# yangye1098/Speech-Denoising-Diffusion-Model-2

Measured on AMD Instinct MI355X. Metric: denoised audio sec/sec, 1000-step UNetModified2 @16kHz, higher is better.
Workload: dtype bf16; 1 GPU; UNetModified2 config_unet.json, linear 1e-6..1e-3, T=1000, 16x16448-sample chunks per GPU, condition_in; model=UNetModified2, global_batch=16, seq_len=16448, parallelism=dp1, lane_rows=16

## Files before the change

speech-denoising-diffusion-model-2_amd/csrc/conv_common.h:

```cpp
#pragma once
#include <cstdlib>

#include "sddm_common.h"

namespace sddm {

template <typename T> struct Frag;
template <> struct Frag<bf16_t> { bf16x8 v; };
template <> struct Frag<f16_t> { f16x8 v; };
template <> struct Frag<float> { f32x4 lo, hi; };

template <typename T> __device__ __forceinline__ Frag<T> load_frag(const char* p);
template <> __device__ __forceinline__ Frag<bf16_t> load_frag<bf16_t>(const char* p) { return {*(const bf16x8*)p}; }
template <> __device__ __forceinline__ Frag<f16_t> load_frag<f16_t>(const char* p) { return {*(const f16x8*)p}; }
template <> __device__ __forceinline__ Frag<float> load_frag<float>(const char* p) {
  return {*(const f32x4*)p, *(const f32x4*)(p + 16)};
}

__device__ __forceinline__ void mfma_frag(f32x4& acc, const Frag<bf16_t>& a, const Frag<bf16_t>& b) {
  acc = __builtin_amdgcn_mfma_f32_16x16x32_bf16(a.v, b.v, acc, 0, 0, 0);
}
__device__ __forceinline__ void mfma_frag(f32x4& acc, const Frag<f16_t>& a, const Frag<f16_t>& b) {
  acc = __builtin_amdgcn_mfma_f32_16x16x32_f16(a.v, b.v, acc, 0, 0, 0);
}
// ... 23 lines not shown

template <typename T>
__device__ __forceinline__ void transform16(char* dst, const char* src, const float* sc, const float* sh, bool gn) {
  *(f32x4*)dst = transform_vec<T>(*(const f32x4*)src, sc, sh, gn);
}

template <typename T> __device__ __forceinline__ void store4(T* p, float a, float b, float c, float d);
template <> __device__ __forceinline__ void store4<float>(float* p, float a, float b, float c, float d) {
  *(f32x4*)p = f32x4{a, b, c, d};
}
template <> __device__ __forceinline__ void store4<bf16_t>(bf16_t* p, float a, float b, float c, float d) {
  *(bf16x4*)p = bf16x4{(bf16_t)a, (bf16_t)b, (bf16_t)c, (bf16_t)d};
}
template <> __device__ __forceinline__ void store4<f16_t>(f16_t* p, float a, float b, float c, float d) {
  *(f16x4*)p = f16x4{(f16_t)a, (f16_t)b, (f16_t)c, (f16_t)d};
}
typedef float f32x2 __attribute__((ext_vector_type(2)));
template <typename T> __device__ __forceinline__ void store4p(T* p, f32x2 a, f32x2 b) { store4<T>(p, a.x, a.y, b.x, b.y); }
template <> __device__ __forceinline__ void store4p<bf16_t>(bf16_t* p, f32x2 a, f32x2 b) {
  typedef bf16_t bf16x2_t __attribute__((ext_vector_type(2)));
  typedef unsigned int u32x2_t __attribute__((ext_vector_type(2)));
  const bf16x2_t x = __builtin_convertvector(a, bf16x2_t), y = __builtin_convertvector(b, bf16x2_t);
  *(u32x2_t*)p = u32x2_t{__builtin_bit_cast(unsigned int, x), __builtin_bit_cast(unsigned int, y)};
}
template <typename T> __device__ __forceinline__ f32x2 unpack2(T a, T b) { return f32x2{to_f32<T>(a), to_f32<T>(b)}; }
template <typename T> __device__ __forceinline__ f32x4 load4(const T* p);
template <> __device__ __forceinline__ f32x4 load4<float>(const float* p) { return *(const f32x4*)p; }
template <> __device__ __forceinline__ f32x4 load4<bf16_t>(const bf16_t* p) {
  const bf16x4 v = *(const bf16x4*)p;
  return f32x4{(float)v[0], (float)v[1], (float)v[2], (float)v[3]};
}
template <> __device__ __forceinline__ f32x4 load4<f16_t>(const f16_t* p) {
  const f16x4 v = *(const f16x4*)p;
  return f32x4{(float)v[0], (float)v[1], (float)v[2], (float)v[3]};
}
template <typename T> __device__ __forceinline__ float round_t(float v) { return to_f32<T>(from_f32<T>(v)); }

}

namespace sddm {

template <int CTRL> __device__ __forceinline__ float dpp_f32(float x) {
  return __builtin_bit_cast(float, __builtin_amdgcn_update_dpp(0, __builtin_bit_cast(int, x), CTRL, 0xF, 0xF, false));
}
__device__ __forceinline__ float row_sum16(float x) {
  x += dpp_f32<0xB1>(x);
// ... 276 lines not shown
```

speech-denoising-diffusion-model-2_amd/csrc/conv_deep.hip:

```cpp
#include "conv_common.h"
#include "conv_tile_cfg.h"
#include "kernels.h"

namespace sddm {

__device__ __attribute__((aligned(256))) unsigned char g_deep_zero[256];

constexpr int kDeepMaxChunks = 10;

#ifdef SDDM_STAMPS_ISSUE
#define DS_W(a) SDDM_STAMP(a, 1)
#define DS_STG(a) SDDM_STAMP(a, 2)
#define DS_ISSUED(a) SDDM_STAMP(a, 3)
#define DS_LANDED(a) SDDM_STAMP(a, 4)
#define DS_XFORM(a) SDDM_STAMP(a, 5)
#define DS_KLOOP(a) SDDM_STAMP(a, 6)
#define DS_STORED(a) do {} while (0)
#define DS_STATS(a) do {} while (0)
#else
#define DS_W(a) do {} while (0)
#define DS_STG(a) do {} while (0)
#define DS_ISSUED(a) SDDM_STAMP(a, 1)
#define DS_LANDED(a) SDDM_STAMP(a, 2)
#define DS_XFORM(a) SDDM_STAMP(a, 3)
// ... 303 lines not shown
      }
      put(wv);
    }
  } else {
    put(wv);
  }
  lds_sync();

  float sn = 0.f, s1[4], s2[4];
#pragma unroll
  for (int i = 0; i < 4; ++i) { s1[i] = 0.f; s2[i] = 0.f; }
  T* out = (T*)a.out + (size_t)b * img_out * gCout + n0 + ec4;
#pragma unroll
  for (int it = 0; it < EIT; ++it) {
    const int p = it * PPI + tid / TPP;
    if (p < npv) {
      const int py = p / gTW, px = p - py * gTW;
      f32x4 s = *(const f32x4*)(red + p * NBP + ec4);
#pragma unroll
      for (int w = 1; w < SLOTS; ++w) s += *(const f32x4*)(red + (w * MT + p) * NBP + ec4);
      float d[4];
#pragma unroll
      for (int i = 0; i < 4; ++i) d[i] = s[i] + idr[it][i];
      store4<T>(out + ((y0 + py) * gWo + (x0 + px)) * gCout, d[0] + bb[0], d[1] + bb[1], d[2] + bb[2], d[3] + bb[3]);
#pragma unroll
      for (int i = 0; i < 4; ++i) {
        s1[i] += d[i];
        s2[i] += d[i] * d[i];
      }
      sn += 1.f;
    }
  }
  DS_STORED(a);
  if (a.stats) {
    auto wred = [](float x) {
      if constexpr (TPP == 4) x += dpp_f32<0x124>(x);
      if constexpr (TPP <= 8) x += dpp_f32<0x128>(x);
      x += __shfl_xor(x, 16);
      return x + __shfl_xor(x, 32);
    };
    const float tn = wred(sn);
    float t1[4], t2[4];
#pragma unroll
    for (int i = 0; i < 4; ++i) { t1[i] = wred(s1[i]); t2[i] = wred(s2[i]); }
    lds_sync();
    float* xs = red;
    if (lane < TPP)
// ... 135 lines not shown
```

speech-denoising-diffusion-model-2_amd/csrc/conv_strip_impl.h:

```cpp
#pragma once
#include <type_traits>

#ifndef SDDM_ABL_STRIP
#define SDDM_ABL_STRIP 0
#endif
#ifndef SDDM_STRIP_WLD
#define SDDM_STRIP_WLD 1
#endif
#ifndef SDDM_STRIP_WREG
#define SDDM_STRIP_WREG 1
#endif

#include "conv_common.h"
#include "conv_tile_cfg.h"
#include "kernels.h"

namespace sddm {

static constexpr ConvShape kStripShapes[] = {
    {-1, 0, 1, 1, 1, 1, 0, 0, 0, 0, 0, 0, 0, 0, 0, 0, 0},
    {32, 0, 16, 128, 256, 128, 32, 0, 32, 0, 0, 0, 1, 0, 256, 16, 0},
    {32, 0, 16, 128, 256, 128, 32, 0, 32, 0, 0, 1, 1, 0, 256, 16, 0},
    {64, 0, 8, 64, 128, 64, 32, 0, 64, 0, 0, 0, 1, 0, 256, 8, 0},
    {32, 0, 16, 64, 128, 64, 64, 0, 64, 32, 0, 2, 1, 0, 256, 16, 0},
// ... 16 lines not shown
    {32, 0, 64, 128, 512, 128, 32, 32, 32, 0, 0, 0, 1, 0, 256, 64, 1},
    {32, 0, 64, 128, 512, 128, 32, 0, 32, 32, 32, 2, 1, 0, 256, 64, 1},
};
static constexpr int kNStripShapes = (int)(sizeof(kStripShapes) / sizeof(kStripShapes[0]));

__host__ inline bool strip_shape_matches(const ConvShape& c, int nblk, int mpi, int SR, const ConvArgs& a) {
  return c.cfg == nblk && c.nw == mpi && c.nb == SR && c.Ho == a.Ho && c.Wo == a.Wo && c.CA == a.CA && c.CB == a.CB &&
         c.Cout == a.Cout && c.RCA == a.RCA && c.RCB == a.RCB && c.res == a.res_mode &&
         c.gn == (a.gamma != nullptr ? 1 : 0) && c.up == (a.upsample ? 1 : 0) && a.n_tiles == c.Ho / SR &&
         a.Hi == (c.up ? c.Ho / 2 : c.Ho) && a.Wi == (c.up ? c.Wo / 2 : c.Wo);
}

template <typename T, int FC, int W, int CIN, int MPI, int RES, bool GN, int SH>
__global__ __launch_bounds__(MPI * 2) void conv_strip_kernel(ConvArgs a, int SR_) {
  constexpr ConvShape SC = kStripShapes[SH];
  constexpr bool CS = SH > 0;
  SDDM_SHAPE_GEO(SC, CS, false, a)
  const int SR = CS ? SC.nb : SR_;
  (void)gTR; (void)gTW; (void)gTX; (void)gRes; (void)gGN; (void)gWo;
  constexpr int NT = MPI * 2;
  constexpr int NWV = NT / 64;
  constexpr int ES = (int)sizeof(T);
  constexpr int NBLK = 16 * FC, FP = 2;
  constexpr int TR = MPI / W, R = 2 * TR + 2;
  constexpr int UPP = CIN * ES / 16;
  constexpr int UPL = ES / 2;
  constexpr int VE = 16 / ES;
  constexpr int PL = ((W + 2) * 16 + 255) / 256 * 256;
  constexpr int SLOT = UPP * PL;
  constexpr int NCK = CIN / 32;
  constexpr int WPL = NBLK * 16;
  constexpr int WPLANES = NCK * 9 * 4 * UPL;
  constexpr int PB = 64 / UPP;
  constexpr int NU = TR * W * UPP;
  constexpr int UPT = NU / NT;
  constexpr int IU = ((TR + 2) * W * UPP + NT - 1) / NT;
  constexpr int RCKM = 4;
  static_assert(UPP >= 1 && UPP <= 64 && (64 % UPP) == 0, "channel units must divide a wave");
  static_assert(NU % NT == 0, "prefetch must split evenly");
  typedef T vec4 __attribute__((ext_vector_type(4)));
  extern __shared__ __attribute__((aligned(16))) char smem[];

  const int tid = threadIdx.x, lane = tid & 63, wave = tid >> 6, g = lane >> 4;
  int strip, b, zb;
  xcd_block<SDDM_XCD_ZIN != 0>(gNT, gCout / NBLK, strip, b, zb);
  const int n0 = zb * NBLK;
// ... 21 lines not shown
#pragma unroll
  for (int k = 0; k < IU; ++k) {
    const int u = min(tid + k * NT, (TR + 2) * W * UPP - 1);
    const int grp = u >> 6, j = u & 63;
    const int pix = grp * PB + (j % PB), q = j / PB, r = pix / W, x = pix % W;
    const int ry = min(max(y0 - 1 + r, 0), H - 1);
    const int sy = gUp ? ry >> 1 : ry, sx = gUp ? x >> 1 : x;
    const int c0 = q * VE;
    const bool fa = c0 < gCA;
    ini[k] = *(const f32x4*)((fa ? srcAb : srcBb) + ((size_t)sy * gWi + sx) * (fa ? gCA : gCB) + (fa ? c0 : c0 - gCA));
  }
  constexpr int WUN = NBLK * WPLANES, WU = (WUN + NT - 1) / NT;
  constexpr bool WLD = SDDM_STRIP_WLD && WU <= 12;
  constexpr int RUN_MAX = RES == 2 ? NBLK * RCKM * 4 * UPL : 0, RU = (RUN_MAX + NT - 1) / NT;
  const int RUN = NBLK * RPLANES;
  f32x4 wst[WLD ? WU : 1], rst[WLD && RU > 0 ? RU : 1];
  if constexpr (WLD) {
#pragma unroll
    for (int i = 0; i < WU; ++i) {
      const int u0 = tid + i * NT, u = u0 < WUN ? u0 : 0;
      const int co = u % NBLK, pl = u / NBLK;
      const char* src;
      if constexpr (ES == 2) {
        src = (const char*)a.wgt_t + ((size_t)pl * gCout + n0 + co) * 16;
      } else {
        const int ck = pl / (9 * 4 * UPL), rem = pl - ck * 9 * 4 * UPL, tap = rem / (4 * UPL), un = rem - tap * 4 * UPL;
        src = (const char*)a.wgt + ((((size_t)(n0 + co) * NCK + ck) * 9 + tap) * 32) * ES + un * 16;
      }
      wst[i] = *(const f32x4*)src;
    }
    if constexpr (RES == 2) {
#pragma unroll
      for (int i = 0; i < RU; ++i) {
        const int u0 = tid + i * NT, u = u0 < RUN ? u0 : 0;
        const int co = u % NBLK, pl = u / NBLK;
        const char* src = ES == 2 ? (const char*)a.res_wgt_t + ((size_t)pl * gCout + n0 + co) * 16
                                  : (const char*)a.res_wgt + ((size_t)(n0 + co) * RC) * ES + pl * 16;
        rst[i] = *(const f32x4*)src;
      }
    }
  } else {
    for (int u0 = wave * 64; u0 < NBLK * WPLANES; u0 += NT) {
      const int u = u0 + lane;
      const int co = u % NBLK, pl = u / NBLK;
      const char* src;
      if constexpr (ES == 2) {
        src = (const char*)a.wgt_t + ((size_t)pl * gCout + n0 + co) * 16;
      } else {
        const int ck = pl / (9 * 4 * UPL), rem = pl - ck * 9 * 4 * UPL, tap = rem / (4 * UPL), un = rem - tap * 4 * UPL;
        src = (const char*)a.wgt + ((((size_t)(n0 + co) * NCK + ck) * 9 + tap) * 32) * ES + un * 16;
      }
      __builtin_amdgcn_global_load_lds((const __attribute__((address_space(1))) void*)src,
                                       (__attribute__((address_space(3))) void*)(wl + u0 * 16), 16, 0, 0);
    }
    if constexpr (RES == 2) {
      for (int u0 = wave * 64; u0 < NBLK * RPLANES; u0 += NT) {
        const int u = u0 + lane;
        const int co = u % NBLK, pl = u / NBLK;
        const char* src = ES == 2 ? (const char*)a.res_wgt_t + ((size_t)pl * gCout + n0 + co) * 16
                                  : (const char*)a.res_wgt + ((size_t)(n0 + co) * RC) * ES + pl * 16;
        __builtin_amdgcn_global_load_lds((const __attribute__((address_space(1))) void*)src,
                                         (__attribute__((address_space(3))) void*)(rw + u0 * 16), 16, 0, 0);
      }
    }
  }
  for (int u = tid; u < R * UPP * 2; u += NT) {
    const int side = u & 1, pl = u >> 1;
    *(f32x4*)(ring + pl * PL + (side ? (W + 1) : 0) * 16) = f32x4{0.f, 0.f, 0.f, 0.f};
  }
  if (gn) gl.finish(gf, b, gCA, gCB, gsc, gsc + CIN);
  __syncthreads();
  const int t_now = a.t_dev ? *a.t_dev : 0;
  const float* trow = a.temb ? a.temb + (size_t)(a.temb_per_b ? b : t_now) * a.temb_ld : a.bias;
  float badd[FC][4];
#pragma unroll
  for (int fc = 0; fc < FC; ++fc)
#pragma unroll
    for (int i = 0; i < 4; ++i) {
      const int co = n0 + fc * 16 + 4 * g + i;
      const float bv = a.bias[co], tv = trow[co];
      badd[fc][i] = bv + (a.temb ? tv : 0.f);
    }
  float sshift;
  {
    const int cs = n0 + (tid % NBLK);
    const float bv = a.bias[cs], tv = trow[cs];
    sshift = bv + (a.temb ? tv : 0.f);
  }
  const int base = ((y0 - 1) % R + R) % R;
#pragma unroll
  for (int k = 0; k < IU; ++k) {
    const int u = tid + k * NT;
    if (u >= (TR + 2) * W * UPP) break;
    const int grp = u >> 6, j = u & 63;
    const int pix = grp * PB + (j % PB), q = j / PB, r = pix / W, x = pix % W;
    const int ry = y0 - 1 + r;
    f32x4 v = ini[k];
    if (ry < 0 || ry >= H) v = f32x4{0.f, 0.f, 0.f, 0.f};
    else if (gn) v = transform_fast<T>(v, gsc + q * VE, gsc + CIN + q * VE);
    *(f32x4*)(ring + ((base + r) % R) * SLOT + q * PL + (x + 1) * 16) = v;
  }

// ... 37 lines not shown
#pragma unroll
    for (int k = 0; k < UPT; ++k) {
      const int ry = min(y0 + j * TR + 1 + pr[k], H - 1);
      const int sy = gUp ? (ry >> 1) : ry;
      dst[k] = *(const f32x4*)(rsrc_[k] + (unsigned)__umul24((unsigned)sy, rstr[k]));
    }
  };
  auto xform_unit = [&](const f32x4 (&src)[UPT], int j, int k) {
    const int ry = y0 + j * TR + 1 + pr[k];
    f32x4 v = src[k];
    if constexpr (GN) v = transform_lds<T>(v, gsc + cq[k], gsc + CIN + cq[k]);
    return ry >= H ? f32x4{0.f, 0.f, 0.f, 0.f} : v;
  };
  auto store_rows = [&](const f32x4 (&tv)[UPT], int j) {
    const int sb = (base + j * TR + 2) % R;
#pragma unroll
    for (int k = 0; k < UPT; ++k) {
      int sl = sb + pr[k];
      sl = sl >= R ? sl - R : sl;
      *(f32x4*)(ring + (int)__umul24(sl, SLOT) + loff[k]) = tv[k];
    }
  };
  T* outb = (T*)a.out + (size_t)b * H * W * gCout;
  const T* resb = RES == 1 ? (const T*)a.res_src + (size_t)b * H * W * gCout : outb;
  auto issue_res1 = [&](vec4 (&dst)[FP][FC], int it) {
#pragma unroll
    for (int fp = 0; fp < FP; ++fp) {
      const int yy = min(y0 + it * TR, H - TR) + prow[fp];
      const unsigned po = (unsigned)(yy * W * gCout) + __umul24((unsigned)pcol[fp], (unsigned)gCout) + n0 + 4 * g;
#pragma unroll
      for (int fc = 0; fc < FC; ++fc) dst[fp][fc] = *(const vec4*)((const char*)resb + (po * ES + fc * 16 * ES));
    }
  };
  const T* rawAb = RES == 2 ? (const T*)a.rawA + (size_t)b * H * W * gRCA : outb;
  const T* rawBb = (RES == 2 && gRCB) ? (const T*)a.rawB + (size_t)b * H * W * gRCB : rawAb;
  auto issue_res2 = [&](Frag<T> (&dst)[RCKM][FP], int it) {
#pragma unroll
    for (int ck = 0; ck < RCKM; ++ck)
#pragma unroll
      for (int fp = 0; fp < FP; ++fp) {
        const int yy = min(y0 + it * TR, H - TR) + prow[fp];
        const int c0 = min(ck, rck - 1) * 32 + g * 8;
        const int pix = yy * W + pcol[fp];
        const T* sp = c0 < gRCA ? rawAb + ((int)__umul24(pix, gRCA) + c0) : rawBb + ((int)__umul24(pix, gRCB) + (c0 - gRCA));
        dst[ck][fp] = load_frag<T>((const char*)sp);
      }
  };

  f32x2 s1[FC][2], s2[FC][2], bp[FC][2];
#pragma unroll
  for (int fc = 0; fc < FC; ++fc)
#pragma unroll
    for (int h = 0; h < 2; ++h) {
      s1[fc][h] = f32x2{0.f, 0.f};
// ... 53 lines not shown
          for (int fp = 0; fp < FP; ++fp)
            if (!(dbg & 8)) mfma_frag(acc[fp][fc], af, bf[fp]);
        }
#pragma unroll
        for (int k = 0; k < UPT; ++k)
          if (decltype(LX)::value && ck * 9 + tap == k * 9 * NCK / UPT) tv[k] = (dbg & 2) ? fill[k] : xform_unit(fill, it + 1, k);
      }
    }
    if constexpr (RES == 2) {
#pragma unroll
      for (int ck = 0; ck < RCKM; ++ck) {
        if (ck >= rck) break;
#pragma unroll
        for (int fc = 0; fc < FC; ++fc) {
          const Frag<T> af = load_planes<T>(rbase + ck * 4 * UPL * WPL + fc * 256, WPL);
#pragma unroll
          for (int fp = 0; fp < FP; ++fp) mfma_frag(acc[fp][fc], af, r2cur[ck][fp]);
        }
      }
    }
#pragma unroll
    for (int fp = 0; fp < FP; ++fp) {
      const unsigned po = (unsigned)((y + prow[fp]) * W * gCout) + __umul24((unsigned)pcol[fp], (unsigned)gCout);
#pragma unroll
      for (int fc = 0; fc < FC; ++fc) {
        const unsigned co = n0 + fc * 16 + 4 * g;
        f32x2 d0 = f32x2{acc[fp][fc][0], acc[fp][fc][1]}, d1 = f32x2{acc[fp][fc][2], acc[fp][fc][3]};
        if constexpr (RES == 1) {
          d0 += unpack2<T>(r1cur[fp][fc][0], r1cur[fp][fc][1]);
          d1 += unpack2<T>(r1cur[fp][fc][2], r1cur[fp][fc][3]);
        }
        if (!(dbg & 128)) store4p<T>((T*)((char*)outb + (po + co) * ES), d0 + bp[fc][0], d1 + bp[fc][1]);
        s1[fc][0] += d0;
        s1[fc][1] += d1;
        s2[fc][0] = __builtin_elementwise_fma(d0, d0, s2[fc][0]);
        s2[fc][1] = __builtin_elementwise_fma(d1, d1, s2[fc][1]);
      }
    }
    if constexpr (decltype(LX)::value) store_rows(tv, it + 1);
    lds_sync();
  };
  issue_rows(rowsA, 1);
  if constexpr (RES == 1) issue_res1(r1A, 0);
  if constexpr (RES == 2) issue_res2(r2A, 0);
  constexpr int NYOUNG = UPT + (RES == 1 ? FP * FC : 0) + (RES == 2 ? RCKM * FP : 0);
  static_assert(NYOUNG < 64, "vmcnt is a 6-bit counter");
  asm volatile("s_waitcnt vmcnt(%0) lgkmcnt(0)\n\ts_barrier" :: "n"(NYOUNG) : "memory");
  if constexpr (WREG) {
#pragma unroll
    for (int tap = 0; tap < 9; ++tap)
#pragma unroll
      for (int fc = 0; fc < FC; ++fc) wreg[tap][fc] = load_planes<T>(abase + tap * 4 * UPL * WPL + fc * 256, WPL);
  }
  SDDM_STAMP(a, 3);
  using yes = std::integral_constant<bool, true>;
  using no = std::integral_constant<bool, false>;
  for (int it = 0; it < iters - 2; it += 2) {
    body(yes{}, yes{}, it, rowsB, rowsA, r1A, r1B, r2A, r2B);
    body(yes{}, yes{}, it + 1, rowsA, rowsB, r1B, r1A, r2B, r2A);
  }
  body(no{}, yes{}, iters - 2, rowsB, rowsA, r1A, r1B, r2A, r2B);
  body(no{}, no{}, iters - 1, rowsA, rowsB, r1B, r1A, r2B, r2A);

  SDDM_STAMP(a, 4);
  if (a.stats) {
    const float nl = (float)(FP * iters) * 16.f;
#pragma unroll
    for (int fc = 0; fc < FC; ++fc)
#pragma unroll
      for (int i = 0; i < 4; ++i) {
        const float t1 = row_sum16(s1[fc][i >> 1][i & 1]), t2 = row_sum16(s2[fc][i >> 1][i & 1]);
        if ((lane & 15) == 0) {
          float* rr = red + ((wave * NBLK) + fc * 16 + 4 * g + i) * 3;
          rr[0] = nl; rr[1] = t1; rr[2] = t2;
        }
      }
    lds_sync();
    if (tid < NBLK) {
      float n = 0.f, u1 = 0.f, u2 = 0.f;
      for (int w = 0; w < NWV; ++w) {
        const float* rr = red + (w * NBLK + tid) * 3;
        n += rr[0]; u1 += rr[1]; u2 += rr[2];
      }
      float* dst = a.stats + (((size_t)b * gNT + strip) * gCout + n0 + tid) * 2;
      dst[0] = (sshift + u1 / n) * n;
      dst[1] = fmaxf(u2 - u1 * u1 / n, 0.f);
    }
  }
  SDDM_STAMP(a, 6);
  SDDM_STAMP(a, 7);
}

template <typename T, int FC, int W, int CIN, int MPI>
static size_t strip_lds(const ConvArgs& a) {
  constexpr int ES = (int)sizeof(T), NBLK = 16 * FC, TR = MPI / W, R = 2 * TR + 2;
  constexpr int UPP = CIN * ES / 16, PL = ((W + 2) * 16 + 255) / 256 * 256;
// ... 63 lines not shown
```

speech-denoising-diffusion-model-2_amd/csrc/conv_tile.hip:

```cpp
#include "conv_common.h"
#include "conv_tile_cfg.h"
#include "kernels.h"

#ifndef SDDM_TILE_WREG
#define SDDM_TILE_WREG 1
#endif

namespace sddm {

template <typename T, bool S2, int WPX, int WCO, int FP, int FC, int MAXU, int SH>
__global__ __launch_bounds__(64 * WPX * WCO) void conv_tile_kernel(ConvArgs a) {
  constexpr int NWV = WPX * WCO, NT = 64 * NWV;
  constexpr int MT = WPX * FP * 16, NB = WCO * FC * 16;
  constexpr int WCH = 576 * NB;
  static_assert(sizeof(T) == 2, "conv_tile is the 16-bit path");
  typedef T vec4 __attribute__((ext_vector_type(4)));
  extern __shared__ __attribute__((aligned(16))) char smem[];
  constexpr ConvShape SC = kTileShapes[SH];
  constexpr bool CS = SH > 0;
  SDDM_SHAPE_GEO(SC, CS, S2, a)

  const int tid = threadIdx.x, lane = tid & 63, g = lane >> 4, c16 = lane & 15, q = lane & 3;
  const int wv = __builtin_amdgcn_readfirstlane(tid >> 6);
  const int wp = wv % WPX, wc = wv / WPX;
  int tile, b, zb;
  xcd_block<SDDM_XCD_ZIN != 0>(gNT, gCout / NB, tile, b, zb);
  const int n0 = zb * NB;
  const int ty = tile / gTX, tx = tile - ty * gTX;
  const int y0 = ty * gTR, x0 = tx * gTW;
  const int npv = gTR * gTW;
  const int Cin = gCA + gCB, nck = Cin / 32, ckA = gCA / 32;
  const int RC = gRCA + gRCB, rck = gRes == 2 ? RC / 32 : 0, rckA = gRCA / 32;
  const int nk = nck + rck;
  const bool gn = gGN, ident = gRes == 1;
  const TileGeo geo = tile_geo(S2, gTR, gTW, MT, rck > 0);
  const int HC = geo.HC, HE = geo.HE, PLB = geo.PLB;
  const int nbuf = nk > 1 ? 2 : 1;
  char* IB = smem;
  char* WB = IB + nbuf * geo.ibb;
  float* gsc = (float*)(WB + nbuf * WCH);
  const float rHC = 1.0f / (float)HC, rTW = 1.0f / (float)gTW;
  const int img_in = gHi * gWi, img_out = gHo * gWo;
  const T* srcA = (const T*)a.srcA + (size_t)b * img_in * gCA;
  const T* srcB = gCB ? (const T*)a.srcB + (size_t)b * img_in * gCB : srcA;
  const T* rawA = rck ? (const T*)a.rawA + (size_t)b * img_out * gRCA : srcA;
  const T* rawB = (rck && gRCB) ? (const T*)a.rawB + (size_t)b * img_out * gRCB : rawA;
  SDDM_STAMP(a, 0);

  GNLoad gl;
  const GNFuse gf{a.gstA, a.gtilesA, a.gntileA, a.gstB, a.gtilesB, a.gntileB, a.gamma, a.beta, a.groups, a.eps};
  gl.issue(gf, b, gCA, gCB, gn, a.bias);
  const int t_now = a.t_dev ? *a.t_dev : 0;
  const float* trow = a.temb ? a.temb + (size_t)(a.temb_per_b ? b : t_now) * a.temb_ld : a.bias;
  const int cw0 = wc * FC * 16, pw0 = wp * FP * 16;
  float bb[FC][4];
#pragma unroll
  for (int fc = 0; fc < FC; ++fc)
#pragma unroll
    for (int i = 0; i < 4; ++i) {
      const int co = n0 + cw0 + fc * 16 + 4 * g + i;
      const float bv = a.bias[co], tv = trow[co];
      bb[fc][i] = bv + (a.temb ? tv : 0.f);
    }
  float sshift;
  {
    const int cs = n0 + (tid % NB);
    const float bv = a.bias[cs], tv = trow[cs];
    sshift = bv + (a.temb ? tv : 0.f);
  }
  int ppy[FP], ppx[FP];
  bool pok[FP];
#pragma unroll
  for (int fp = 0; fp < FP; ++fp) {
    int p = pw0 + fp * 16 + c16;
    pok[fp] = p < npv;
    if (!pok[fp]) p = 0;
    ppy[fp] = fdivi(p, rTW);
    ppx[fp] = p - ppy[fp] * gTW;
  }
  vec4 r1[FP][FC];
  {
    const T* rs = ident ? (const T*)a.res_src + (size_t)b * img_out * gCout : srcA;
#pragma unroll
    for (int fp = 0; fp < FP; ++fp) {
      const int po = ident ? ((y0 + ppy[fp]) * gWo + (x0 + ppx[fp])) * gCout : 0;
#pragma unroll
      for (int fc = 0; fc < FC; ++fc) r1[fp][fc] = *(const vec4*)(rs + po + (ident ? n0 + cw0 + fc * 16 + 4 * g : 0));
    }
  }
  int spx[MAXU], sof[MAXU];
#pragma unroll
  for (int j = 0; j < MAXU; ++j) {
    const int u = tid + j * NT, s = u >> 2;
    const int hy = fdivi(s, rHC), hx = s - hy * HC;
    int iy, ix, slot;
    bool ok;
    if (S2) {
      iy = 2 * y0 - 1 + hy; ix = 2 * x0 - 1 + hx;
      ok = iy >= 0 && iy < gHi && ix >= 0 && ix < gWi;
      slot = hy * HC + ((hx & 1) ? HE + (hx >> 1) : (hx >> 1));
    } else {
      iy = y0 - 1 + hy; ix = x0 - 1 + hx;
      ok = iy >= 0 && iy < gHo && ix >= 0 && ix < gWo;
      if (gUp) { iy >>= 1; ix >>= 1; }
      slot = s;
    }
    spx[j] = ok ? iy * gWi + ix : -1;
    sof[j] = u < geo.nu3 ? q * PLB + ((slot ^ (q << 1)) << 4) : -1;
  }

// ... 6 lines not shown
#pragma unroll
      for (int j = 0; j < MAXU; ++j) rr[j] = *(const f32x4*)(base + (spx[j] < 0 ? 0 : spx[j] * cs));
    } else {
      const int r = k - nck;
      const bool fa = r < rckA;
      const T* base = (fa ? rawA + r * 32 : rawB + (r - rckA) * 32) + q * 8;
      const int cs = fa ? gRCA : gRCB;
#pragma unroll
      for (int j = 0; j < MAXU; ++j) {
        const int p = (tid + j * NT) >> 2;
        const int py = fdivi(p, rTW), px = p - py * gTW;
        rr[j] = *(const f32x4*)(base + (p < npv ? ((y0 + py) * gWo + (x0 + px)) * cs : 0));
      }
    }
  };
  auto issue_w = [&](int k, int buf) {
    char* dst = WB + buf * WCH;
    const bool res = k >= nck;
    const int nw = (res ? 4 : 36) * NB;
    const char* ws = res ? (const char*)a.res_wgt_t + (size_t)(k - nck) * 4 * gCout * 16
                         : (const char*)a.wgt_t + (size_t)k * 36 * gCout * 16;
    for (int u0 = wv * 64; u0 < nw; u0 += NT) {
      const int u = u0 + lane, r = u / NB, co = u - r * NB;
      glds16(ws + ((size_t)r * gCout + n0 + co) * 16, dst + u0 * 16);
    }
  };
  constexpr bool WR = SDDM_TILE_WREG && (SH > 0 || FP * FC <= 6);
  constexpr int WU = (36 * NB + NT - 1) / NT;
  f32x4 wr[WR ? WU : 1];
  auto load_w = [&](int k) {
    const bool res = k >= nck;
    const int nw = (res ? 4 : 36) * NB;
    const char* ws = res ? (const char*)a.res_wgt_t + (size_t)(k - nck) * 4 * gCout * 16
                         : (const char*)a.wgt_t + (size_t)k * 36 * gCout * 16;
#pragma unroll
    for (int i = 0; i < WU; ++i) {
      const int u = tid + i * NT, uu = u < nw ? u : 0, r = uu / NB, co = uu - r * NB;
      wr[i] = *(const f32x4*)(ws + ((size_t)r * gCout + n0 + co) * 16);
    }
  };
  auto store_w = [&](int k, int buf) {
    const int nw = (k >= nck ? 4 : 36) * NB;
    char* dst = WB + buf * WCH;
#pragma unroll
    for (int i = 0; i < WU; ++i) {
      const int u = tid + i * NT;
      if (u < nw) *(f32x4*)(dst + u * 16) = wr[i];
    }
  };
  auto transform = [&](int k, int buf) {
    char* ib = IB + buf * geo.ibb;
    if (k < nck) {
      float sc[8], sh[8];
      if (gn) {
        const int c = k * 32 + q * 8;
#pragma unroll
        for (int j = 0; j < 8; j += 4) {
          const f32x4 s4 = *(const f32x4*)(gsc + c + j), h4 = *(const f32x4*)(gsc + Cin + c + j);
#pragma unroll
          for (int i = 0; i < 4; ++i) { sc[j + i] = s4[i]; sh[j + i] = h4[i]; }
        }
// ... 86 lines not shown
      if (k + 1 < nk) {
        if (!(dbg & 4)) load_raw(k + 1);
        if (!(dbg & 32)) load_w(k + 1);
      }
      if (!(dbg & 8)) mma(k, cur);
      if (k + 1 < nk) {
        if (!(dbg & 2)) transform(k + 1, nxt);
        if (!(dbg & 32)) store_w(k + 1, nxt);
      }
      lds_sync();
    } else {
      if (k + 1 < nk) {
        if (!(dbg & 4)) load_raw(k + 1);
        if (!(dbg & 32)) issue_w(k + 1, nxt);
      }
      if (!(dbg & 8)) mma(k, cur);
      if (k + 1 < nk && !(dbg & 2)) transform(k + 1, nxt);
      dma_sync();
    }
  }
  SDDM_STAMP(a, 4);

  T* out = (T*)a.out + (size_t)b * img_out * gCout;
  float s1[FC][4], s2[FC][4], nl = 0.f;
#pragma unroll
  for (int fc = 0; fc < FC; ++fc)
#pragma unroll
    for (int i = 0; i < 4; ++i) { s1[fc][i] = 0.f; s2[fc][i] = 0.f; }
#pragma unroll
  for (int fp = 0; fp < FP; ++fp) {
    if (!pok[fp]) continue;
    nl += 1.f;
    const int po = ((y0 + ppy[fp]) * gWo + (x0 + ppx[fp])) * gCout;
#pragma unroll
    for (int fc = 0; fc < FC; ++fc) {
      const int co = n0 + cw0 + fc * 16 + 4 * g;
      float d[4];
#pragma unroll
      for (int i = 0; i < 4; ++i) d[i] = acc[fp][fc][i] + (ident ? to_f32<T>(r1[fp][fc][i]) : 0.f);
      if (!(dbg & 128)) store4<T>(out + po + co, d[0] + bb[fc][0], d[1] + bb[fc][1], d[2] + bb[fc][2], d[3] + bb[fc][3]);
#pragma unroll
      for (int i = 0; i < 4; ++i) {
        s1[fc][i] += d[i];
        s2[fc][i] += d[i] * d[i];
      }
    }
  }
  SDDM_STAMP(a, 5);
  if (a.stats) {
    float* red = (float*)IB;
    const float nr = row_sum16(nl);
#pragma unroll
    for (int fc = 0; fc < FC; ++fc)
#pragma unroll
      for (int i = 0; i < 4; ++i) {
        const float t1 = row_sum16(s1[fc][i]), t2 = row_sum16(s2[fc][i]);
        if (c16 == 0) {
          float* e = red + (wp * NB + cw0 + fc * 16 + 4 * g + i) * 3;
          e[0] = nr; e[1] = t1; e[2] = t2;
        }
      }
    lds_sync();
    if (tid < NB) {
      float n = 0.f, t1 = 0.f, t2 = 0.f;
#pragma unroll
      for (int w = 0; w < WPX; ++w) {
        const float* e = red + (w * NB + tid) * 3;
        n += e[0]; t1 += e[1]; t2 += e[2];
      }
      const int co = tid;
      const float mean = sshift + t1 / n;
      float* dst = a.stats + (((size_t)b * gNT + tile) * gCout + n0 + co) * 2;
      dst[0] = mean * n;
      dst[1] = fmaxf(t2 - t1 * t1 / n, 0.f);
    }
  }
  SDDM_STAMP(a, 6);
  SDDM_STAMP(a, 7);
}

template <int I>
// ... 76 lines not shown
```

speech-denoising-diffusion-model-2_amd/csrc/kernels.hip:

```cpp
#include "sddm_common.h"
#include "kernels.h"
#include "conv_common.h"
#include <algorithm>
#include <type_traits>

namespace sddm {


__global__ __launch_bounds__(256) void embed_kernel(EmbedArgs a) {
  __shared__ float enc[128];
  __shared__ float h1[512];
  __shared__ float h2[128];
  const int r = blockIdx.x, tid = threadIdx.x, D = a.dim, H = a.dim / 2, D4 = 4 * a.dim;
  float nl;
  if (a.noise_levels) nl = a.noise_levels[r];
  else if (a.time_step_mode) nl = (float)r;
  else nl = a.table[r];
  if (tid < D) {
    const float arg = __fmul_rn(nl, a.emb_vec[tid % H]);
    enc[tid] = tid < H ? sinf(arg) : cosf(arg);
  }
  __syncthreads();
  for (int j = tid; j < D4; j += blockDim.x) {
    float s = a.b1[j];
// ... 73 lines not shown
    a.scale[(size_t)b * C + c] = (float)sc;
    a.shift[(size_t)b * C + c] = (float)((double)a.beta[c] - mean * sc);
  }
}

hipError_t launch_gn_finalize(const GNArgs& a, hipStream_t s) {
  hipLaunchKernelGGL(gn_finalize_kernel, dim3(a.G, a.B), dim3(256), 0, s, a);
  return hipGetLastError();
}

template <typename T>
__global__ __launch_bounds__(256) void conv_in_kernel(ConvInArgs a) {
  constexpr int CO = 32;
  constexpr int IMAX = 6 * 130;
  constexpr int NFR = 8;
  __shared__ float img[2][IMAX];
  __shared__ float xs_red[4][CO][2];
  const int b = blockIdx.y, f0 = blockIdx.x * a.TR, tid = threadIdx.x;
  const int lane = tid & 63, wave = tid >> 6, g = lane >> 4;
  if (a.t_dev && blockIdx.x == 0 && blockIdx.y == 0 && tid == 0) *a.t_dev -= 1;
  SDDM_STAMP_AT(a, 0, blockIdx.x + blockIdx.y * (a.F / a.TR));
  const int S = a.S, F = a.F, W = a.W, IW = W + 2, IH = a.TR + 2;
  constexpr int KPL = sizeof(T) == 4 ? 5 : 8;
  float bias[2][4];
#pragma unroll
  for (int fc = 0; fc < 2; ++fc)
#pragma unroll
    for (int i = 0; i < 4; ++i) bias[fc][i] = a.bias[fc * 16 + 4 * g + i];
  float wf[2][KPL];
#pragma unroll
  for (int j = 0; j < KPL; ++j) {
    const int k = sizeof(T) == 4 ? 4 * j + g : 8 * g + j;
    const int kk = k < 18 ? k : 0;
#pragma unroll
    for (int fc = 0; fc < 2; ++fc) wf[fc][j] = a.w[(fc * 16 + (lane & 15)) * 18 + kk];
  }
  {
    const float* c0 = a.cond + (size_t)b * a.N;
    const float* x0 = a.x + (size_t)b * a.N;
    constexpr int IPT = (IMAX + 255) / 256;
    float cv[IPT], xv[IPT];
#pragma unroll
    for (int k = 0; k < IPT; ++k) {
      const int i = min(tid + 256 * k, IH * IW - 1);
      const int r = i / IW, c = i - r * IW, f = f0 - 1 + r, w = c - 1;
      const bool ok = f >= 0 && f < F && w >= 0 && w < W;
      const int n = ok ? f * S + w : 0;
      cv[k] = c0[n];
      xv[k] = x0[n];
      cv[k] = ok ? cv[k] : 0.f;
      xv[k] = ok ? xv[k] : 0.f;
    }
#pragma unroll
    for (int k = 0; k < IPT; ++k) {
      const int i = tid + 256 * k;
      if (i < IH * IW) { img[0][i] = cv[k]; img[1][i] = xv[k]; }
    }
  }
// ... 7 lines not shown
    koff[j] = ch * IMAX + (tap / 3) * IW + (tap % 3);
#pragma unroll
    for (int fc = 0; fc < 2; ++fc) wf[fc][j] = kok[j] ? wf[fc][j] : 0.f;
  }
  f16x8 wh[2], wl[2];
#pragma unroll
  for (int fc = 0; fc < 2; ++fc)
#pragma unroll
    for (int j = 0; j < 8; ++j) {
      const float v = j < KPL ? wf[fc][j] : 0.f;
      wh[fc][j] = (f16_t)v;
      wl[fc][j] = (f16_t)(v - (float)wh[fc][j]);
    }
  f32x2 st1[2][2], st2[2][2], bp[2][2];
#pragma unroll
  for (int fc = 0; fc < 2; ++fc)
#pragma unroll
    for (int h = 0; h < 2; ++h) {
      st1[fc][h] = f32x2{0.f, 0.f};
      st2[fc][h] = f32x2{0.f, 0.f};
      bp[fc][h] = f32x2{bias[fc][2 * h], bias[fc][2 * h + 1]};
    }
  const float rW = 1.0f / (float)W;
  __syncthreads();
  SDDM_STAMP_AT(a, 1, blockIdx.x + blockIdx.y * (a.F / a.TR));
  const float* imgf = &img[0][0];
#pragma unroll 2
  for (int fr = 0; fr < NFR; ++fr) {
    const int p = wave * (NFR * 16) + fr * 16 + (lane & 15);
    const int r = fdivi(p, rW), w = p - r * W;
    const int pb = r * IW + w;
    float xv[KPL];
#pragma unroll
    for (int j = 0; j < KPL; ++j) xv[j] = kok[j] ? imgf[pb + koff[j]] : 0.f;
    f32x4 acc[2];
    if constexpr (sizeof(T) == 4) {
#pragma unroll
      for (int fc = 0; fc < 2; ++fc) {
        acc[fc] = f32x4{0.f, 0.f, 0.f, 0.f};
#pragma unroll
        for (int j = 0; j < KPL; ++j) acc[fc] = __builtin_amdgcn_mfma_f32_16x16x4f32(wf[fc][j], xv[j], acc[fc], 0, 0, 0);
      }
    } else if constexpr (std::is_same<T, bf16_t>::value) {
      f16x8 xh;
#pragma unroll
      for (int j = 0; j < 8; ++j) xh[j] = (f16_t)(j < KPL ? xv[j] : 0.f);
#pragma unroll
      for (int fc = 0; fc < 2; ++fc)
        acc[fc] = __builtin_amdgcn_mfma_f32_16x16x32_f16(wh[fc], xh, f32x4{0.f, 0.f, 0.f, 0.f}, 0, 0, 0);
    } else {
      f16x8 xh, xl;
#pragma unroll
      for (int j = 0; j < 8; ++j) {
        const float v = j < KPL ? xv[j] : 0.f;
        xh[j] = (f16_t)v;
        xl[j] = (f16_t)(v - (float)xh[j]);
      }
#pragma unroll
      for (int fc = 0; fc < 2; ++fc) {
        acc[fc] = __builtin_amdgcn_mfma_f32_16x16x32_f16(wh[fc], xh, f32x4{0.f, 0.f, 0.f, 0.f}, 0, 0, 0);
        acc[fc] = __builtin_amdgcn_mfma_f32_16x16x32_f16(wh[fc], xl, acc[fc], 0, 0, 0);
        acc[fc] = __builtin_amdgcn_mfma_f32_16x16x32_f16(wl[fc], xh, acc[fc], 0, 0, 0);
      }
    }
    T* op = (T*)a.out + (((size_t)b * F + f0 + r) * W + w) * CO;
#pragma unroll
    for (int fc = 0; fc < 2; ++fc) {
      const f32x2 d0 = f32x2{acc[fc][0], acc[fc][1]}, d1 = f32x2{acc[fc][2], acc[fc][3]};
      st1[fc][0] += d0;
      st1[fc][1] += d1;
      st2[fc][0] = __builtin_elementwise_fma(d0, d0, st2[fc][0]);
      st2[fc][1] = __builtin_elementwise_fma(d1, d1, st2[fc][1]);
      store4p<T>(op + fc * 16 + 4 * g, d0 + bp[fc][0], d1 + bp[fc][1]);
    }
  }
  SDDM_STAMP_AT(a, 2, blockIdx.x + blockIdx.y * (a.F / a.TR));
#pragma unroll
  for (int fc = 0; fc < 2; ++fc)
#pragma unroll
    for (int i = 0; i < 4; ++i) {
      const float t1 = row_sum16(st1[fc][i >> 1][i & 1]);
      const float t2 = row_sum16(st2[fc][i >> 1][i & 1]);
      if ((lane & 15) == 0) {
        xs_red[wave][fc * 16 + 4 * g + i][0] = t1;
        xs_red[wave][fc * 16 + 4 * g + i][1] = t2;
      }
    }
  lds_sync();
  SDDM_STAMP_AT(a, 3, blockIdx.x + blockIdx.y * (a.F / a.TR));
  if (tid < CO) {
    const float n = (float)(a.TR * W);
    float S1 = 0.f, S2 = 0.f;
#pragma unroll
    for (int w4 = 0; w4 < 4; ++w4) { S1 += xs_red[w4][tid][0]; S2 += xs_red[w4][tid][1]; }
    float* dst = a.stats + (((size_t)b * (a.F / a.TR) + blockIdx.x) * CO + tid) * 2;
    dst[0] = a.bias[tid] * n + S1;
    dst[1] = fmaxf(S2 - S1 * S1 / n, 0.f);
  }
  SDDM_STAMP_AT(a, 6, blockIdx.x + blockIdx.y * (a.F / a.TR));
  SDDM_STAMP_AT(a, 7, blockIdx.x + blockIdx.y * (a.F / a.TR));
}

hipError_t launch_conv_in(int dtype, const ConvInArgs& a, int B, hipStream_t s) {
  if (a.Cout != 32 || a.TR * a.W != 512 || a.F % a.TR || (a.TR + 2) * (a.W + 2) > 6 * 130) return hipErrorInvalidValue;
  dim3 grid(a.F / a.TR, B);
  if (dtype == DT_F32) hipLaunchKernelGGL(conv_in_kernel<float>, grid, dim3(256), 0, s, a);
  else if (dtype == DT_BF16) hipLaunchKernelGGL(conv_in_kernel<bf16_t>, grid, dim3(256), 0, s, a);
  else hipLaunchKernelGGL(conv_in_kernel<f16_t>, grid, dim3(256), 0, s, a);
// ... 305 lines not shown
```

Measured before the change: 25.07 audio_s/s.

## Permute output channels to pair fragments into 16-byte stores with streaming hints

Remaps which output channels each MFMA fragment computes, so a lane holds 8 adjacent channels across two fragment columns. The conv_in and strip kernels can then emit one 16-byte store where they previously issued two 8-byte stores. Weight, bias, residual and stats indexing are permuted to match. Separately, 16-bit output stores go through buffer or atomic-relaxed stores with a cache-policy bit (write-through or streaming) in the strip and conv_in paths, to cut write-back traffic. The risks are extra register pressure from holding paired values and possible cache side effects when the next layer reads these outputs.

```diff
diff --git a/speech-denoising-diffusion-model-2_amd/csrc/conv_common.h b/speech-denoising-diffusion-model-2_amd/csrc/conv_common.h
--- a/speech-denoising-diffusion-model-2_amd/csrc/conv_common.h
+++ b/speech-denoising-diffusion-model-2_amd/csrc/conv_common.h
@@ -69,6 +69,67 @@
   typedef unsigned int u32x2_t __attribute__((ext_vector_type(2)));
   const bf16x2_t x = __builtin_convertvector(a, bf16x2_t), y = __builtin_convertvector(b, bf16x2_t);
   *(u32x2_t*)p = u32x2_t{__builtin_bit_cast(unsigned int, x), __builtin_bit_cast(unsigned int, y)};
+}
+#ifndef SDDM_WT_STRIP
+#define SDDM_WT_STRIP 1
+#endif
+#ifndef SDDM_WT_TILE
+#define SDDM_WT_TILE 0
+#endif
+#ifndef SDDM_WT_DEEP
+#define SDDM_WT_DEEP 0
+#endif
+#ifndef SDDM_WT_IN
+#define SDDM_WT_IN 1
+#endif
+typedef __attribute__((address_space(1))) unsigned long long gu64_t;
+__device__ __forceinline__ void store8b_wt(void* p, unsigned long long v) {
+  __hip_atomic_store((gu64_t*)p, v, __ATOMIC_RELAXED, __HIP_MEMORY_SCOPE_AGENT);
+}
+template <bool WT, typename T> __device__ __forceinline__ void store4(T* p, float a, float b, float c, float d) {
+  if constexpr (WT && sizeof(T) == 2) {
+    typedef T vec4 __attribute__((ext_vector_type(4)));
+    store8b_wt(p, __builtin_bit_cast(unsigned long long, vec4{(T)a, (T)b, (T)c, (T)d}));
+  } else {
+    store4<T>(p, a, b, c, d);
+  }
+}
+template <bool WT, typename T> __device__ __forceinline__ void store4p(T* p, f32x2 a, f32x2 b) {
+  if constexpr (WT && sizeof(T) == 2) {
+    typedef T vec2 __attribute__((ext_vector_type(2)));
+    typedef unsigned int u32x2_t __attribute__((ext_vector_type(2)));
+    const vec2 x = __builtin_convertvector(a, vec2), y = __builtin_convertvector(b, vec2);
+    store8b_wt(p, __builtin_bit_cast(unsigned long long,
+                                     u32x2_t{__builtin_bit_cast(unsigned int, x), __builtin_bit_cast(unsigned int, y)}));
+  } else {
+    store4p<T>(p, a, b);
+  }
+}
+#ifndef SDDM_ST16_IN
+#define SDDM_ST16_IN 1
+#endif
+#ifndef SDDM_ST16_STRIP
+#define SDDM_ST16_STRIP 1
+#endif
+#ifndef SDDM_ST16_TILE
+#define SDDM_ST16_TILE 0
+#endif
+__host__ __device__ constexpr int pair_channel(int fc, int r) { return 8 * (r / 4) + 4 * (fc & 1) + r % 4 + 32 * (fc / 2); }
+template <bool ST16> __device__ constexpr int slab_channel(int c) { return ST16 ? pair_channel(c >> 4, c & 15) : c; }
+typedef unsigned int u32x4_t __attribute__((ext_vector_type(4)));
+__device__ __forceinline__ __amdgpu_buffer_rsrc_t out_rsrc(void* base, unsigned bytes) {
+  return __builtin_amdgcn_make_buffer_rsrc(base, 0, (int)bytes, 0x00020000);
+}
+template <typename T> __device__ __forceinline__ unsigned int pack2(f32x2 a) {
+  typedef T vec2 __attribute__((ext_vector_type(2)));
+  return __builtin_bit_cast(unsigned int, __builtin_convertvector(a, vec2));
+}
+template <bool WT, typename T>
+__device__ __forceinline__ void store8p(char* base, __amdgpu_buffer_rsrc_t rs, unsigned off, f32x2 a, f32x2 b, f32x2 c, f32x2 d) {
+  static_assert(sizeof(T) == 2, "16-byte stores of 8 channels: 16-bit storage types");
+  const u32x4_t v = u32x4_t{pack2<T>(a), pack2<T>(b), pack2<T>(c), pack2<T>(d)};
+  if constexpr (WT) __builtin_amdgcn_raw_buffer_store_b128(v, rs, (int)off, 0, 16);
+  else *(u32x4_t*)(base + off) = v;
 }
 template <typename T> __device__ __forceinline__ f32x2 unpack2(T a, T b) { return f32x2{to_f32<T>(a), to_f32<T>(b)}; }
 template <typename T> __device__ __forceinline__ f32x4 load4(const T* p);
diff --git a/speech-denoising-diffusion-model-2_amd/csrc/conv_deep.hip b/speech-denoising-diffusion-model-2_amd/csrc/conv_deep.hip
--- a/speech-denoising-diffusion-model-2_amd/csrc/conv_deep.hip
+++ b/speech-denoising-diffusion-model-2_amd/csrc/conv_deep.hip
@@ -349,7 +349,7 @@
       float d[4];
 #pragma unroll
       for (int i = 0; i < 4; ++i) d[i] = s[i] + idr[it][i];
-      store4<T>(out + ((y0 + py) * gWo + (x0 + px)) * gCout, d[0] + bb[0], d[1] + bb[1], d[2] + bb[2], d[3] + bb[3]);
+      store4<SDDM_WT_DEEP != 0, T>(out + ((y0 + py) * gWo + (x0 + px)) * gCout, d[0] + bb[0], d[1] + bb[1], d[2] + bb[2], d[3] + bb[3]);
 #pragma unroll
       for (int i = 0; i < 4; ++i) {
         s1[i] += d[i];
diff --git a/speech-denoising-diffusion-model-2_amd/csrc/conv_strip_impl.h b/speech-denoising-diffusion-model-2_amd/csrc/conv_strip_impl.h
--- a/speech-denoising-diffusion-model-2_amd/csrc/conv_strip_impl.h
+++ b/speech-denoising-diffusion-model-2_amd/csrc/conv_strip_impl.h
@@ -62,6 +62,7 @@
   constexpr int NWV = NT / 64;
   constexpr int ES = (int)sizeof(T);
   constexpr int NBLK = 16 * FC, FP = 2;
+  constexpr bool ST16 = SDDM_ST16_STRIP != 0 && ES == 2 && FC % 2 == 0;
   constexpr int TR = MPI / W, R = 2 * TR + 2;
   constexpr int UPP = CIN * ES / 16;
   constexpr int UPL = ES / 2;
@@ -129,7 +130,7 @@
       const int co = u % NBLK, pl = u / NBLK;
       const char* src;
       if constexpr (ES == 2) {
-        src = (const char*)a.wgt_t + ((size_t)pl * gCout + n0 + co) * 16;
+        src = (const char*)a.wgt_t + ((size_t)pl * gCout + n0 + slab_channel<ST16>(co)) * 16;
       } else {
         const int ck = pl / (9 * 4 * UPL), rem = pl - ck * 9 * 4 * UPL, tap = rem / (4 * UPL), un = rem - tap * 4 * UPL;
         src = (const char*)a.wgt + ((((size_t)(n0 + co) * NCK + ck) * 9 + tap) * 32) * ES + un * 16;
@@ -141,7 +142,7 @@
       for (int i = 0; i < RU; ++i) {
         const int u0 = tid + i * NT, u = u0 < RUN ? u0 : 0;
         const int co = u % NBLK, pl = u / NBLK;
-        const char* src = ES == 2 ? (const char*)a.res_wgt_t + ((size_t)pl * gCout + n0 + co) * 16
+        const char* src = ES == 2 ? (const char*)a.res_wgt_t + ((size_t)pl * gCout + n0 + slab_channel<ST16>(co)) * 16
                                   : (const char*)a.res_wgt + ((size_t)(n0 + co) * RC) * ES + pl * 16;
         rst[i] = *(const f32x4*)src;
       }
@@ -152,7 +153,7 @@
       const int co = u % NBLK, pl = u / NBLK;
       const char* src;
       if constexpr (ES == 2) {
-        src = (const char*)a.wgt_t + ((size_t)pl * gCout + n0 + co) * 16;
+        src = (const char*)a.wgt_t + ((size_t)pl * gCout + n0 + slab_channel<ST16>(co)) * 16;
       } else {
         const int ck = pl / (9 * 4 * UPL), rem = pl - ck * 9 * 4 * UPL, tap = rem / (4 * UPL), un = rem - tap * 4 * UPL;
         src = (const char*)a.wgt + ((((size_t)(n0 + co) * NCK + ck) * 9 + tap) * 32) * ES + un * 16;
@@ -164,7 +165,7 @@
       for (int u0 = wave * 64; u0 < NBLK * RPLANES; u0 += NT) {
         const int u = u0 + lane;
         const int co = u % NBLK, pl = u / NBLK;
-        const char* src = ES == 2 ? (const char*)a.res_wgt_t + ((size_t)pl * gCout + n0 + co) * 16
+        const char* src = ES == 2 ? (const char*)a.res_wgt_t + ((size_t)pl * gCout + n0 + slab_channel<ST16>(co)) * 16
                                   : (const char*)a.res_wgt + ((size_t)(n0 + co) * RC) * ES + pl * 16;
         __builtin_amdgcn_global_load_lds((const __attribute__((address_space(1))) void*)src,
                                          (__attribute__((address_space(3))) void*)(rw + u0 * 16), 16, 0, 0);
@@ -184,7 +185,7 @@
   for (int fc = 0; fc < FC; ++fc)
 #pragma unroll
     for (int i = 0; i < 4; ++i) {
-      const int co = n0 + fc * 16 + 4 * g + i;
+      const int co = n0 + slab_channel<ST16>(fc * 16 + 4 * g + i);
       const float bv = a.bias[co], tv = trow[co];
       badd[fc][i] = bv + (a.temb ? tv : 0.f);
     }
@@ -268,14 +269,17 @@
     }
   };
   T* outb = (T*)a.out + (size_t)b * H * W * gCout;
+  [[maybe_unused]] const __amdgpu_buffer_rsrc_t ors = out_rsrc(outb, (unsigned)(H * W * gCout) * (unsigned)ES);
   const T* resb = RES == 1 ? (const T*)a.res_src + (size_t)b * H * W * gCout : outb;
   auto issue_res1 = [&](vec4 (&dst)[FP][FC], int it) {
 #pragma unroll
     for (int fp = 0; fp < FP; ++fp) {
       const int yy = min(y0 + it * TR, H - TR) + prow[fp];
-      const unsigned po = (unsigned)(yy * W * gCout) + __umul24((unsigned)pcol[fp], (unsigned)gCout) + n0 + 4 * g;
-#pragma unroll
-      for (int fc = 0; fc < FC; ++fc) dst[fp][fc] = *(const vec4*)((const char*)resb + (po * ES + fc * 16 * ES));
+      const unsigned po = (unsigned)(yy * W * gCout) + __umul24((unsigned)pcol[fp], (unsigned)gCout) + n0 +
+                          slab_channel<ST16>(4 * g);
+#pragma unroll
+      for (int fc = 0; fc < FC; ++fc)
+        dst[fp][fc] = *(const vec4*)((const char*)resb + (po * ES + (slab_channel<ST16>(fc * 16) * ES)));
     }
   };
   const T* rawAb = RES == 2 ? (const T*)a.rawA + (size_t)b * H * W * gRCA : outb;
@@ -375,6 +379,7 @@
 #pragma unroll
     for (int fp = 0; fp < FP; ++fp) {
       const unsigned po = (unsigned)((y + prow[fp]) * W * gCout) + __umul24((unsigned)pcol[fp], (unsigned)gCout);
+      [[maybe_unused]] f32x2 pv0, pv1;
 #pragma unroll
       for (int fc = 0; fc < FC; ++fc) {
         const unsigned co = n0 + fc * 16 + 4 * g;
@@ -383,7 +388,18 @@
           d0 += unpack2<T>(r1cur[fp][fc][0], r1cur[fp][fc][1]);
           d1 += unpack2<T>(r1cur[fp][fc][2], r1cur[fp][fc][3]);
         }
-        if (!(dbg & 128)) store4p<T>((T*)((char*)outb + (po + co) * ES), d0 + bp[fc][0], d1 + bp[fc][1]);
+        if constexpr (ST16) {
+          if (fc & 1) {
+            if (!(dbg & 128))
+              store8p<SDDM_WT_STRIP != 0, T>((char*)outb, ors, (po + n0 + (fc / 2) * 32 + 8 * g) * ES, pv0, pv1,
+                                             d0 + bp[fc][0], d1 + bp[fc][1]);
+          } else {
+            pv0 = d0 + bp[fc][0];
+            pv1 = d1 + bp[fc][1];
+          }
+        } else {
+          if (!(dbg & 128)) store4p<SDDM_WT_STRIP != 0, T>((T*)((char*)outb + (po + co) * ES), d0 + bp[fc][0], d1 + bp[fc][1]);
+        }
         s1[fc][0] += d0;
         s1[fc][1] += d1;
         s2[fc][0] = __builtin_elementwise_fma(d0, d0, s2[fc][0]);
@@ -424,7 +440,7 @@
       for (int i = 0; i < 4; ++i) {
         const float t1 = row_sum16(s1[fc][i >> 1][i & 1]), t2 = row_sum16(s2[fc][i >> 1][i & 1]);
         if ((lane & 15) == 0) {
-          float* rr = red + ((wave * NBLK) + fc * 16 + 4 * g + i) * 3;
+          float* rr = red + ((wave * NBLK) + slab_channel<ST16>(fc * 16 + 4 * g + i)) * 3;
           rr[0] = nl; rr[1] = t1; rr[2] = t2;
         }
       }
diff --git a/speech-denoising-diffusion-model-2_amd/csrc/conv_tile.hip b/speech-denoising-diffusion-model-2_amd/csrc/conv_tile.hip
--- a/speech-denoising-diffusion-model-2_amd/csrc/conv_tile.hip
+++ b/speech-denoising-diffusion-model-2_amd/csrc/conv_tile.hip
@@ -14,6 +14,7 @@
   constexpr int MT = WPX * FP * 16, NB = WCO * FC * 16;
   constexpr int WCH = 576 * NB;
   static_assert(sizeof(T) == 2, "conv_tile is the 16-bit path");
+  constexpr bool ST16 = SDDM_ST16_TILE != 0 && FC % 2 == 0;
   typedef T vec4 __attribute__((ext_vector_type(4)));
   extern __shared__ __attribute__((aligned(16))) char smem[];
   constexpr ConvShape SC = kTileShapes[SH];
@@ -58,7 +59,7 @@
   for (int fc = 0; fc < FC; ++fc)
 #pragma unroll
     for (int i = 0; i < 4; ++i) {
-      const int co = n0 + cw0 + fc * 16 + 4 * g + i;
+      const int co = n0 + cw0 + slab_channel<ST16>(fc * 16 + 4 * g + i);
       const float bv = a.bias[co], tv = trow[co];
       bb[fc][i] = bv + (a.temb ? tv : 0.f);
     }
@@ -85,7 +86,7 @@
     for (int fp = 0; fp < FP; ++fp) {
       const int po = ident ? ((y0 + ppy[fp]) * gWo + (x0 + ppx[fp])) * gCout : 0;
 #pragma unroll
-      for (int fc = 0; fc < FC; ++fc) r1[fp][fc] = *(const vec4*)(rs + po + (ident ? n0 + cw0 + fc * 16 + 4 * g : 0));
+      for (int fc = 0; fc < FC; ++fc) r1[fp][fc] = *(const vec4*)(rs + po + (ident ? n0 + cw0 + slab_channel<ST16>(fc * 16 + 4 * g) : 0));
     }
   }
   int spx[MAXU], sof[MAXU];
@@ -138,7 +139,7 @@
                          : (const char*)a.wgt_t + (size_t)k * 36 * gCout * 16;
     for (int u0 = wv * 64; u0 < nw; u0 += NT) {
       const int u = u0 + lane, r = u / NB, co = u - r * NB;
-      glds16(ws + ((size_t)r * gCout + n0 + co) * 16, dst + u0 * 16);
+      glds16(ws + ((size_t)r * gCout + n0 + slab_channel<ST16>(co)) * 16, dst + u0 * 16);
     }
   };
   constexpr bool WR = SDDM_TILE_WREG && (SH > 0 || FP * FC <= 6);
@@ -152,7 +153,7 @@
 #pragma unroll
     for (int i = 0; i < WU; ++i) {
       const int u = tid + i * NT, uu = u < nw ? u : 0, r = uu / NB, co = uu - r * NB;
-      wr[i] = *(const f32x4*)(ws + ((size_t)r * gCout + n0 + co) * 16);
+      wr[i] = *(const f32x4*)(ws + ((size_t)r * gCout + n0 + slab_channel<ST16>(co)) * 16);
     }
   };
   auto store_w = [&](int k, int buf) {
@@ -285,6 +286,7 @@
   SDDM_STAMP(a, 4);
 
   T* out = (T*)a.out + (size_t)b * img_out * gCout;
+  [[maybe_unused]] const __amdgpu_buffer_rsrc_t ors = out_rsrc(out, (unsigned)(img_out * gCout) * (unsigned)sizeof(T));
   float s1[FC][4], s2[FC][4], nl = 0.f;
 #pragma unroll
   for (int fc = 0; fc < FC; ++fc)
@@ -295,13 +297,26 @@
     if (!pok[fp]) continue;
     nl += 1.f;
     const int po = ((y0 + ppy[fp]) * gWo + (x0 + ppx[fp])) * gCout;
+    [[maybe_unused]] f32x2 pv0, pv1;
 #pragma unroll
     for (int fc = 0; fc < FC; ++fc) {
       const int co = n0 + cw0 + fc * 16 + 4 * g;
       float d[4];
 #pragma unroll
       for (int i = 0; i < 4; ++i) d[i] = acc[fp][fc][i] + (ident ? to_f32<T>(r1[fp][fc][i]) : 0.f);
-      if (!(dbg & 128)) store4<T>(out + po + co, d[0] + bb[fc][0], d[1] + bb[fc][1], d[2] + bb[fc][2], d[3] + bb[fc][3]);
+      if constexpr (ST16) {
+        const f32x2 o0 = f32x2{d[0] + bb[fc][0], d[1] + bb[fc][1]}, o1 = f32x2{d[2] + bb[fc][2], d[3] + bb[fc][3]};
+        if (fc & 1) {
+          if (!(dbg & 128))
+            store8p<SDDM_WT_TILE != 0, T>((char*)out, ors, (unsigned)(po + n0 + cw0 + (fc / 2) * 32 + 8 * g) * (unsigned)sizeof(T),
+                                          pv0, pv1, o0, o1);
+        } else {
+          pv0 = o0;
+          pv1 = o1;
+        }
+      } else {
+        if (!(dbg & 128)) store4<SDDM_WT_TILE != 0, T>(out + po + co, d[0] + bb[fc][0], d[1] + bb[fc][1], d[2] + bb[fc][2], d[3] + bb[fc][3]);
+      }
 #pragma unroll
       for (int i = 0; i < 4; ++i) {
         s1[fc][i] += d[i];
@@ -319,7 +334,7 @@
       for (int i = 0; i < 4; ++i) {
         const float t1 = row_sum16(s1[fc][i]), t2 = row_sum16(s2[fc][i]);
         if (c16 == 0) {
-          float* e = red + (wp * NB + cw0 + fc * 16 + 4 * g + i) * 3;
+          float* e = red + (wp * NB + cw0 + slab_channel<ST16>(fc * 16 + 4 * g + i)) * 3;
           e[0] = nr; e[1] = t1; e[2] = t2;
         }
       }
diff --git a/speech-denoising-diffusion-model-2_amd/csrc/kernels.hip b/speech-denoising-diffusion-model-2_amd/csrc/kernels.hip
--- a/speech-denoising-diffusion-model-2_amd/csrc/kernels.hip
+++ b/speech-denoising-diffusion-model-2_amd/csrc/kernels.hip
@@ -119,18 +119,20 @@
   SDDM_STAMP_AT(a, 0, blockIdx.x + blockIdx.y * (a.F / a.TR));
   const int S = a.S, F = a.F, W = a.W, IW = W + 2, IH = a.TR + 2;
   constexpr int KPL = sizeof(T) == 4 ? 5 : 8;
+  constexpr bool ST16 = SDDM_ST16_IN != 0 && sizeof(T) == 2;
+  auto chan = [](int fc, int r) { return ST16 ? pair_channel(fc, r) : fc * 16 + r; };
   float bias[2][4];
 #pragma unroll
   for (int fc = 0; fc < 2; ++fc)
 #pragma unroll
-    for (int i = 0; i < 4; ++i) bias[fc][i] = a.bias[fc * 16 + 4 * g + i];
+    for (int i = 0; i < 4; ++i) bias[fc][i] = a.bias[chan(fc, 4 * g + i)];
   float wf[2][KPL];
 #pragma unroll
   for (int j = 0; j < KPL; ++j) {
     const int k = sizeof(T) == 4 ? 4 * j + g : 8 * g + j;
     const int kk = k < 18 ? k : 0;
 #pragma unroll
-    for (int fc = 0; fc < 2; ++fc) wf[fc][j] = a.w[(fc * 16 + (lane & 15)) * 18 + kk];
+    for (int fc = 0; fc < 2; ++fc) wf[fc][j] = a.w[chan(fc, lane & 15) * 18 + kk];
   }
   {
     const float* c0 = a.cond + (size_t)b * a.N;
@@ -184,6 +186,8 @@
       bp[fc][h] = f32x2{bias[fc][2 * h], bias[fc][2 * h + 1]};
     }
   const float rW = 1.0f / (float)W;
+  T* const oimg = (T*)a.out + (size_t)b * F * W * CO;
+  [[maybe_unused]] const __amdgpu_buffer_rsrc_t ors = out_rsrc(oimg, (unsigned)(F * W * CO) * (unsigned)sizeof(T));
   __syncthreads();
   SDDM_STAMP_AT(a, 1, blockIdx.x + blockIdx.y * (a.F / a.TR));
   const float* imgf = &img[0][0];
@@ -226,6 +230,7 @@
       }
     }
     T* op = (T*)a.out + (((size_t)b * F + f0 + r) * W + w) * CO;
+    f32x2 ov[2][2];
 #pragma unroll
     for (int fc = 0; fc < 2; ++fc) {
       const f32x2 d0 = f32x2{acc[fc][0], acc[fc][1]}, d1 = f32x2{acc[fc][2], acc[fc][3]};
@@ -233,8 +238,13 @@
       st1[fc][1] += d1;
       st2[fc][0] = __builtin_elementwise_fma(d0, d0, st2[fc][0]);
       st2[fc][1] = __builtin_elementwise_fma(d1, d1, st2[fc][1]);
-      store4p<T>(op + fc * 16 + 4 * g, d0 + bp[fc][0], d1 + bp[fc][1]);
-    }
+      ov[fc][0] = d0 + bp[fc][0];
+      ov[fc][1] = d1 + bp[fc][1];
+      if constexpr (!ST16) store4p<SDDM_WT_IN != 0, T>(op + fc * 16 + 4 * g, ov[fc][0], ov[fc][1]);
+    }
+    if constexpr (ST16)
+      store8p<SDDM_WT_IN != 0, T>((char*)oimg, ors, (unsigned)(((f0 + r) * W + w) * CO + 8 * g) * (unsigned)sizeof(T),
+                                  ov[0][0], ov[0][1], ov[1][0], ov[1][1]);
   }
   SDDM_STAMP_AT(a, 2, blockIdx.x + blockIdx.y * (a.F / a.TR));
 #pragma unroll
@@ -244,8 +254,8 @@
       const float t1 = row_sum16(st1[fc][i >> 1][i & 1]);
       const float t2 = row_sum16(st2[fc][i >> 1][i & 1]);
       if ((lane & 15) == 0) {
-        xs_red[wave][fc * 16 + 4 * g + i][0] = t1;
-        xs_red[wave][fc * 16 + 4 * g + i][1] = t2;
+        xs_red[wave][chan(fc, 4 * g + i)][0] = t1;
+        xs_red[wave][chan(fc, 4 * g + i)][1] = t2;
       }
     }
   lds_sync();
```

New measurement: 25.52 audio_s/s, median of 6. 1.02x the previous value.
